# mwhoffman/pybo

Hardware: AMD Instinct MI355X
Metric: BO-step wall-clock (GP fit + 1e6-candidate acq sweep) at N obs; steps/sec (higher is better)
Workload: dtype f64

## Files before the change

### pybo_amd/csrc/api.hip

```cpp
#include <math.h>
#include <stdio.h>
#include <stdlib.h>
#include <string.h>

#include <algorithm>
#include <cmath>
#include <functional>
#include <new>
#include <type_traits>

#include "gpx_internal.h"
#include "gpx_diag.h"
#include "acq_core.h"
#include "ehvi_math.h"
#include "mes_math.h"
#include "kg_math.h"

using namespace gpx;

static thread_local std::string g_create_err;

#define HIPCHK(h, call)                                                                     \
    do {                                                                                    \
        hipError_t e_ = (call);                                                             \
// ... 93 lines not shown
}

enum { SHIP = 0, DIAG = 1 };
struct Option {
    const char* name;
    int diag;
    int64_t lo, hi;
    const char* bad;
    void (*set)(gpx_handle* h, int64_t v);
    bool (*ok)(int64_t v) = nullptr;
    const char* bad_ok = nullptr;
};
template <int gpx_handle::*F>
static void store(gpx_handle* h, int64_t v) { h->*F = (int)v; }
static bool mult128(int64_t v) { return v % 128 == 0; }
static const int64_t BIG = INT64_MAX;
static const char* const TG = "chol_tg*: out of range";
static const char* const TRTRI = "trtri_ahead*: out of range";
static const char* const XBG = "x_bg*: out of range";
static const Option kOptions[] = {
    {"chunk", SHIP, 128, BIG, "chunk must be a positive multiple of 128", [](gpx_handle* h, int64_t v) { h->chunk = v; }, mult128},
    {"super_m", SHIP, 1, 16, "super_m must be 1, 2, 4, 8 or 16", store<&gpx_handle::super_m>, [](int64_t v) { return (v & (v - 1)) == 0; }},
    {"tile_order", SHIP, -1, 31, "tile_order: -1 (by size) or bits 0-1 tile map (0..3), bits 2-4 k-loop schedule (1 .. 7)",
     store<&gpx_handle::tile_order>, [](int64_t v) { return v == -1 || v >= 4; }},
    {"sweep_cache", SHIP, -1, 1, "sweep_cache must be 1, 0 or -1",
     [](gpx_handle* h, int64_t v) { h->cache_on = (v == 1); if (v < 0) { h->cache_valid = false; h->npend = 0; } }},
    {"prune", SHIP, -1, 1, "prune must be -1 (by size and gate), 0 (never) or 1 (wherever legal)", store<&gpx_handle::prune>},
    {"prune_keep", DIAG, 0, 1, "prune_keep must be 0 or 1", store<&gpx_handle::prune_keep>},
    {"prune_bound", DIAG, -1, 2, "prune_bound must be -1 (by guard), 0 (generic kernel), 1 (matrix-pipe kernel) or 2 (fp32 matrix-pipe kernel)", store<&gpx_handle::prune_bound>},
    {"bound_fact", DIAG, 0, 1, "bound_fact must be 0 (the fp32 bound kernel never takes its factorised form) or 1 (by its guard)", store<&gpx_handle::bound_fact>},
    {"prune_rows", DIAG, -1, 1000000, "prune_rows must be -1 (by size), 0 (no second bound) or a number of block rows", store<&gpx_handle::prune_rows>},
    {"sweep_cols", SHIP, -1, 128, "sweep_cols must be -1 (by size), 128, 64 or 32", store<&gpx_handle::sweep_cols>,
     [](int64_t v) { return v == -1 || v == 128 || v == 64 || v == 32; }},
    {"prune_seeds", DIAG, 0, 1000000, "prune_seeds must be 0 (by the rule) or a number of seeds", store<&gpx_handle::prune_seeds>},
    {"short_map", DIAG, -1, 1, "short_map must be -1 (by size), 0 (never) or 1 (wherever tile map 3 is in use)", store<&gpx_handle::short_map>},
    {"chol_w", SHIP, 0, 8, "chol_w must be 0 (by size) or in [2, 8]", store<&gpx_handle::chol_w>, [](int64_t v) { return v != 1; }},
    {"chol_tg", SHIP, -1, 1000000000, TG, store<&gpx_handle::chol_tg>, [](int64_t v) { return v == 0 || v == 1; }, "chol_tg must be 0 or 1"},
    {"chol_tg_chunks", DIAG, -1, 1000000000, TG, store<&gpx_handle::tg_chunks>},
    {"chol_tg_grid", DIAG, -1, 1000000000, TG, store<&gpx_handle::tg_grid>},
    {"chol_tg_trace", DIAG, -1, 1000000000, TG, store<&gpx_handle::tg_trace>},
    {"chol_tg_isolate", DIAG, -1, 1000000000, TG, store<&gpx_handle::tg_isolate>},
    {"chol_tg_nap", DIAG, -1, 1000000000, TG, [](gpx_handle* h, int64_t v) { h->tg_nap = (int)std::max<int64_t>(0, std::min<int64_t>(127, v)); }},
    {"chol_tg_tmo_ms", SHIP, -1, 1000000000, TG, store<&gpx_handle::tg_tmo_ms>},
    {"chol_tg_min", SHIP, -1, 1000000000, TG, [](gpx_handle* h, int64_t v) { h->tg_min = (int)std::max<int64_t>(1, v); }},
    {"chol_tg_max", SHIP, -1, 1000000000, TG, [](gpx_handle* h, int64_t v) { h->tg_max = (int)std::max<int64_t>(1, v); }},
    {"chol_tg_db", SHIP, -1, 1000000000, TG, [](gpx_handle* h, int64_t v) { h->tg_db = (v < 0) ? -1 : (v != 0 ? 1 : 0); }},
    {"chol_tg_db_max", SHIP, -1, 1000000000, TG, [](gpx_handle* h, int64_t v) { h->tg_db_max = (int)std::max<int64_t>(0, v); }},
    {"chol_tg_fuse", SHIP, -1, 1000000000, TG, [](gpx_handle* h, int64_t v) { h->tg_fuse = (v != 0) ? 1 : 0; }},
    {"trtri_ahead", SHIP, 0, 1000000, TRTRI, [](gpx_handle* h, int64_t v) { h->trtri_ahead = (v != 0) ? 1 : 0; }},
    {"trtri_ahead_min", SHIP, 0, 1000000, TRTRI, [](gpx_handle* h, int64_t v) { h->trtri_ahead_min = (int)std::max<int64_t>(4, v); }},
    {"chol_fuse", SHIP, 0, 1, "chol_fuse must be 0 or 1", store<&gpx_handle::chol_fuse>},
    {"chol_graph", SHIP, 0, 1, "chol_graph must be 0 or 1", store<&gpx_handle::chol_graph>},
    {"chol_merge", SHIP, 0, 100000, "chol_merge: 0 (off) or a minimum number of block rows", store<&gpx_handle::chol_merge>},
    {"chol_rl", SHIP, 0, 1, "chol_rl must be 0 or 1", store<&gpx_handle::chol_rl>},
    {"x_skip", DIAG, 0, 7, "x_skip: bits 0..2", store<&gpx_handle::x_skip>},
    {"x_bg", DIAG, 0, 10000000, XBG, store<&gpx_handle::x_bg>},
    {"x_bg_lds", DIAG, 0, 10000000, XBG, store<&gpx_handle::x_bg_lds>},
    {"x_bg_iters", DIAG, 0, 10000000, XBG, store<&gpx_handle::x_bg_iters>},
    {"x_rff", DIAG, 0, 1, "x_rff must be 0 (by size) or 1 (the round-3 kernel)", [](gpx_handle*, int64_t v) { gpx::g_rff_variant = (int)v; }},
    {"grad_form", SHIP, 0, 2, "grad_form must be 0 (auto), 1 (two passes) or 2 (one pass)", store<&gpx_handle::grad_form>},
    {"grad_rb_cs", DIAG, 0, 65536, "grad_rb_cs must be a multiple of 128 (0 = default)", store<&gpx_handle::grad_rb_cs>, mult128},
    {"grad_kernel", SHIP, -1, 1, "grad_kernel must be -1 (auto), 0 or 1", store<&gpx_handle::grad_kernel>},
    {"trtri_left", SHIP, 0, 1, "trtri_left must be 0 or 1", store<&gpx_handle::trtri_left>},
    {"refine_inverse", SHIP, 0, 1, "refine_inverse must be 0 or 1", [](gpx_handle* h, int64_t v) { h->refine_inverse = (v != 0); }},
    {"eager_inverse", SHIP, 0, 1, "eager_inverse must be 0 or 1", [](gpx_handle* h, int64_t v) { h->eager_inverse = (v != 0); }},
};
// ... 968 lines not shown
        if (list.idx != w.idx) launch_sel_remap(s, w.idx, list.idx, list.n);
        launch_sel_scatter(s, list.idx, vals, list.n, out, nullptr);
    }
    *done = M;
    return GPX_OK;
}

static int plain_rest(const SelectOps& ops, const double* dXc, int64_t done, int64_t chunk, int64_t M, double* out, double* mu, double* s2) {
    const int64_t chunk1 = std::min(chunk, M);
    int rc;
    if (done > 0 && done < chunk1) {
        if ((rc = ops.exact(dXc, done, chunk1, out, mu, s2))) return rc;
        done = chunk1;
    }
    return done < M ? ops.exact(dXc, done, M, out, mu, s2) : GPX_OK;
}

static int second_bound(gpx_handle* h, const PruneWs& w, int64_t chunk, int sweep_order, double p0, SelectList& list) {
    hipStream_t s = h->stream;
    gpx_handle::PruneRecord& rec = h->prune_rec;
    const int64_t Np = h->Np, M = rec.M, Gg = rec.Gg, cap = rec.cap, nsurv = list.n;
    const int nP = (int)(Np / NB);
    int nR = 0;
    if (h->prune_rows > 0) nR = (int)std::min<int64_t>(std::min<int64_t>(h->prune_rows, nP), h->N / NB);
    else if (h->prune_rows < 0 && M >= PRUNE_MIN_M && nP >= PRUNE_ROWS_MIN_NP && nsurv > Gg) nR = std::max(1, nP / PRUNE_ROWS_DIV);
    if (nR <= 0 || nsurv <= 0) return GPX_OK;
    int64_t nsurv2 = 0;
    {
        Span sp(h, T_BOUND);
        for (int64_t j0 = 0; j0 < nsurv; j0 += chunk) {
            const int64_t valid = std::min(chunk, nsurv - j0);
            const int64_t cols = (valid + TBH - 1) / TBH * TBH;
            launch_cross_gram(s, h->dXs, (int64_t)nR * NB, h->N, (int)h->d, w.Xg, j0, nsurv, cols, h->dinvell, h->kernel_id, h->rho, h->dKs, Np);
            launch_sweep_trmm(s, h->dU, Np, nR, h->dKs, chunk, cols, h->da, h->dQp, h->dPp, chunk, sweep_order, h->super_m, h->dclk, h->short_map);
            launch_prune_ub2(s, h->dQp, chunk, nR, j0, valid, w.idx, w.dots, w.sc, h->rho, h->bias, p0, w.ub2, h->prune_keep ? w.qR : nullptr);
        }
    }
    {
        Span sp(h, T_ACQ);
        launch_sel_compact(s, w.ub2, nsurv, 1, w.st, w.sc + 5, w.blk2, cap, w.Xg, (int)h->d, w.idx2, w.Xg2);
        HIPCHK(h, hipMemcpyAsync(&nsurv2, w.blk2 + sel_blocks(nsurv), 8, hipMemcpyDeviceToHost, s));
    }
    HIPCHK(h, hipStreamSynchronize(s));
    rec.nR = nR, rec.nsurv2 = nsurv2;
    rec.ub2 = w.ub2, rec.idx2 = w.idx2, rec.qR = h->prune_keep ? w.qR : nullptr;
    list = {w.Xg2, w.idx2, nsurv2};
    return GPX_OK;
}

static int sweep_core(gpx_handle* h, int acq_id, const double* params, int nparams, const double* dXc,
                      int64_t M, int64_t k, double* top_val, int64_t* top_idx, double* d_acq,
                      double* d_mu, double* d_s2) {
    h->prune_rec = gpx_handle::PruneRecord();
    if (!h->fitted) return fail(h, GPX_ESTATE, "sweep: model is not fitted");
    if (!dXc || M < 1) return fail(h, GPX_EARG, "sweep: need M >= 1 candidates");
    int rc;
    if ((rc = check_acq(h, "sweep", acq_id, params, nparams, 0, true)) || (rc = check_topk(h, "sweep", k, top_val, top_idx))) return rc;
    HIPCHK(h, hipSetDevice(h->device));
    if ((rc = ensure_inverse(h))) return rc;
    hipStream_t s = h->stream;
    const int64_t Np = h->Np;
    const int nP = (int)(Np / NB);
    const int64_t chunk = sweep_chunk(h, M);
    if ((rc = ensure(h, h->dKs, h->cap_ks, Np * chunk))) return rc;
    if ((rc = ensure(h, h->dQp, h->cap_part, (int64_t)nP * chunk * 2))) return rc;
    h->dPp = h->dQp + (int64_t)nP * chunk;
    const bool selection_only = !d_acq && !d_mu && !d_s2;
// ... 9 lines not shown
    if (kg) {
        if ((rc = kg_prepare(h, params, nparams / (int)h->d, kb))) return rc;
        if ((rc = ensure(h, h->dkgw, h->cap_kgw, (int64_t)NB * chunk))) return rc;
    }
    double* cq = nullptr;
    double* cp = nullptr;
    if (h->cache_on) {
        spec_cancel(h);
        h->cache_valid = false;
        h->npend = 0;
        if ((rc = ensure(h, h->dcZ, h->cap_cz, M * h->d))) return rc;
        if ((rc = ensure(h, h->dcq, h->cap_cq, 2 * M))) return rc;
        h->dcp = h->dcq + h->cap_cq / 2;
        cq = h->dcq;
        cp = h->dcp;
        if (dXc != h->dcZ)
            HIPCHK(h, hipMemcpyAsync(h->dcZ, dXc, (size_t)M * h->d * 8, hipMemcpyDeviceToDevice, s));
    }

    const int sweep_order = h->tile_order >= 0 ? h->tile_order : (Np / NB < 32 ? 7 : 19);

    auto run_chunks = [&](const double* X, int64_t mb, int64_t me, double* out, double* mu, double* s2) -> int {
        for (int64_t m0 = mb; m0 < me; m0 += chunk) {
            const int64_t valid = std::min(chunk, me - m0);
            const int64_t cols = (valid + TBH - 1) / TBH * TBH;
            {
                Span sp(h, T_XGRAM);
                launch_cross_gram(s, h->dXs, Np, h->N, (int)h->d, X, m0, me, cols, h->dinvell, h->kernel_id,
                                  h->rho, h->dKs, Np);
            }
            {
                Span sp(h, T_TRMM);
                launch_sweep_trmm(s, h->dU, Np, nP, h->dKs, chunk, cols, h->da, h->dQp, h->dPp, chunk, sweep_order, h->super_m, h->dclk, h->short_map,
                                  valid, h->sweep_cols);
            }
            h->tacc[T_NLAUNCH] += 1.0;
            h->tacc[T_FLOP] += (double)h->N * (double)h->N * (double)valid;
            {
                Span sp(h, T_ACQ);
                if (kg) {
                    launch_kg_cross(s, kb.B, Np, h->dKs, Np, cols, h->dkgw, chunk);
                    launch_acq_kg(s, h->dQp, h->dPp, chunk, nP, m0, valid, h->rho, h->bias, h->sn2, h->kernel_id, (int)h->d, X, h->dinvell,
                                  kb.As, kb.m, kb.al, h->dkgw, chunk, out, mu, s2, cq, cp);
                } else if (mes) launch_acq_mes(s, h->dQp, h->dPp, chunk, nP, m0, valid, h->rho, h->bias, ys, out, mu, s2, cq, cp);
                else launch_acq(s, h->dQp, h->dPp, chunk, nP, m0, valid, h->rho, h->bias, acq_id, p0, out, mu, s2, cq, cp);
            }
        }
        return GPX_OK;
    };

    gpx_handle::PruneRecord& rec = h->prune_rec;
    PruneWs w;
    KeepWs kw = {};
    SelectOps ops;
    ops.exact = run_chunks;
    ops.gate = [&](int64_t Gg, double* value, bool* go) -> int {
        run_chunks(dXc, 0, Gg, d_acq, nullptr, w.gs2);
        launch_prune_mean(s, w.gs2, Gg, w.sc + 4);
        double mean_s2 = 0.0;
        HIPCHK(h, hipMemcpyAsync(&mean_s2, w.sc + 4, 8, hipMemcpyDeviceToHost, s));
        HIPCHK(h, hipStreamSynchronize(s));
        *go = mean_s2 >= h->rho * PRUNE_GATE_S2;
        *value = mean_s2;
        return GPX_OK;
    };
    ops.bound = [&](double* ub, int64_t done) -> int {
        const bool bound_mfma = h->prune_bound != 0 && bound_mfma_ks(h->kernel_id, (int)h->d) > 0;
// ... 1216 lines not shown
```

### pybo_amd/csrc/gemm_core.h

```cpp
#pragma once
#include <hip/hip_runtime.h>
#include <stdint.h>
#include <type_traits>

namespace gpx {

typedef double d4 __attribute__((ext_vector_type(4)));
typedef double d2 __attribute__((ext_vector_type(2)));

constexpr int TB = 128;
constexpr int BK = 16;
constexpr int LDT = TB + 16;
constexpr int GEMM_THREADS = 256;
constexpr int GEMM_LDS_F64 = 2 * 2 * BK * LDT;
constexpr int GEMM_LDS_BYTES = GEMM_LDS_F64 * 8;

template <int NJ>
__device__ __forceinline__ void acc_zero(d4 (&acc)[4][NJ]) {
#pragma unroll
    for (int i = 0; i < 4; ++i)
#pragma unroll
        for (int j = 0; j < NJ; ++j) acc[i][j] = (d4){0.0, 0.0, 0.0, 0.0};
}

// ... 473 lines not shown
        };
        frag(0, 0);
#pragma unroll
        for (int kk = 0; kk < G; ++kk) {
            if (kk + 1 < G) {
                frag((kk + 1) & 1, kk + 1);
                __builtin_amdgcn_sched_group_barrier(0x100, 8, 0);
            }
#pragma unroll
            for (int i = 0; i < 4; ++i)
#pragma unroll
                for (int j = 0; j < 4; ++j)
                    acc[i][j] = __builtin_amdgcn_mfma_f64_16x16x4f64(a[kk & 1][i], b[kk & 1][j], acc[i][j], 0, 0, NEGA ? 1 : 0);
            __builtin_amdgcn_sched_group_barrier(0x008, 16, 0);
            if (FILL && kk < 4) {
                if (kk == 0) issue(img, std::integral_constant<int, 0>{}, std::integral_constant<int, 2>{});
                if (kk == 1) issue(img, std::integral_constant<int, 2>{}, std::integral_constant<int, 4>{});
                if (kk == 2) issue(img, std::integral_constant<int, 4>{}, std::integral_constant<int, 6>{});
                if (kk == 3) issue(img, std::integral_constant<int, 6>{}, std::integral_constant<int, 8>{});
                __builtin_amdgcn_sched_group_barrier(0x020, 4, 0);
            }
        }
        asm volatile("" ::: "memory");
        if (FILL) {
            bump();
            asm volatile("s_waitcnt vmcnt(0) lgkmcnt(0)" ::: "memory");
            __builtin_amdgcn_s_barrier();
        }
    };
    int kt = 0;
    for (; kt + 1 < nk; ++kt) step(kt, std::true_type{});
    step(kt, std::false_type{});
    if (PRIO) __builtin_amdgcn_s_setprio(PRIO - 1);
    __builtin_amdgcn_s_barrier();
}

constexpr int GEMM_W_IMG_F64 = 2 * 16 * 64;

template <int NIMG, int PRIO = 1, bool NEGA = false, bool ILV = false, int AUX = 0, bool TRI = false>
__device__ __forceinline__ void gemm_tile_128_w(d4 (&acc)[4][4], const double* __restrict__ A, int64_t lda,
                                                const double* __restrict__ B, int64_t ldb, int k_lo, int k_hi,
                                                double* smem) {
    constexpr int BKW = 16, G = 4;
    const int lane = threadIdx.x & 63;
    const int w = __builtin_amdgcn_readfirstlane(threadIdx.x >> 6);
    const int wm = w >> 1, wn = w & 1;
    const int nk = (k_hi - k_lo) / BKW;
    if (nk <= 0) return;
    double* mine = smem + w * (NIMG * GEMM_W_IMG_F64);
    const char* Abase = reinterpret_cast<const char*>(A + (int64_t)k_lo * lda);
    const char* Bbase = reinterpret_cast<const char*>(B + (int64_t)k_lo * ldb);
    const int lp = lane >> 4, lr = (lane >> 3) & 1, lc = lane & 7;
    const int colA = (ILV ? (2 * lp + wm) * 16 : wm * 64 + 16 * lp) + 2 * lc, colB = wn * 64 + 16 * lp + 2 * lc;
    const int voA = (int)(((int64_t)lr * lda + colA) * 8), voB = (int)(((int64_t)lr * ldb + colB) * 8);
    const int soA = (int)(2 * lda * 8), soB = (int)(2 * ldb * 8);
    auto issue = [&](int img, auto q0c, auto q1c) {
        constexpr int Q0 = decltype(q0c)::value, Q1 = decltype(q1c)::value;
        double* As = mine + img * GEMM_W_IMG_F64;
        double* Bs = As + 16 * 64;
        __amdgpu_buffer_rsrc_t rA = __builtin_amdgcn_make_buffer_rsrc((void*)Abase, 0, -1, 0x00020000);
        __amdgpu_buffer_rsrc_t rB = __builtin_amdgcn_make_buffer_rsrc((void*)Bbase, 0, -1, 0x00020000);
#pragma unroll
        for (int q = Q0; q < Q1; ++q) {
            __builtin_amdgcn_raw_ptr_buffer_load_lds(rA, (gemm_lds_ptr)(As + q * 128), 16, voA, q * soA, 0, AUX);
            __builtin_amdgcn_raw_ptr_buffer_load_lds(rB, (gemm_lds_ptr)(Bs + q * 128), 16, voB, q * soB, 0, AUX);
        }
// ... 178 lines not shown
```

### pybo_amd/csrc/gpx_internal.h

```cpp
#pragma once
#include <hip/hip_runtime.h>
#include <stdint.h>
#include <string>
#include <vector>

#include "../../include/gpx.h"
#include "prune_hint.h"
#include "ws_layout.h"

namespace gpx {

constexpr int DMAX_RFF = DMAX;
constexpr int DMAX_RFF_RESIDENT = 64;
constexpr int TOPK_MAX = 4096;
constexpr int TOPK_PASS = 64;

enum Timer {
    T_GRAM = 0, T_CHOL, T_TRTRI, T_ALPHA, T_XGRAM, T_TRMM, T_ACQ, T_RFF, T_NLAUNCH, T_FLOP, T_COPY, T_APPEND,
    T_RANK1, T_RFFSWEEP, T_RFFOPS, T_TGFALL, T_SCLK, T_RFFCLK, T_AHEAD, T_BOUND, T_BATCH, T_JOINT, T_COUNT
};

struct EventPair { hipEvent_t a, b; int slot; };

struct EnsBatchMember {
    const double *cq, *cp, *invell;
    double *qp, *V, *cross, *scal, *xs;
    double rho, bias, sn2;
};

}

struct CholGraphKey {
    int64_t Np;
    int w, rl, merge, fuse;
    const void *S, *R, *T, *U, *flag;
    hipStream_t s2, s3, s4;
};

struct gpx_handle {
    int device = 0;
// ... 116 lines not shown
        int64_t M = 0, k = 0, G = 0, Gg = 0, done = 0, cap = 0, nsurv = 0;
        double gate = 0.0;
        bool hinted = false;
        const double* ub = nullptr;
        const int64_t* idx = nullptr;
        const double* sc = nullptr;
    };
    struct PruneRecord : SelectRecord {
        const int* st = nullptr;
        int bound_kernel = -1;
        bool kept = false;
        int nR = 0;
        int64_t nsurv2 = 0;
        const double *qR = nullptr, *ub2 = nullptr;
        const int64_t* idx2 = nullptr;
    } prune_rec;
    struct EnsPruneRecord : SelectRecord {
        int n = 0;
        const double* delta = nullptr;
    } ens_rec;
    struct ConPruneRecord : SelectRecord {
        int nc = 0;
    } con_rec;
    gpx::PruneHint prune_hint, ens_hint;
    int prune_keep = 0;
    int prune_bound = -1;
#ifdef GPX_BOUND32_NOFACT
    int bound_fact = 0;
#else
    int bound_fact = 1;
#endif
    int prune_rows = -1;
    int sweep_cols = -1;
    int prune_seeds = 0;
    int short_map = -1;
    char* dkeep = nullptr;
    int64_t cap_keep = 0;

    const double* app_w = nullptr;
    bool cache_on = false;
    bool cache_valid = false;
    int64_t cache_M = 0;
    double* dcZ = nullptr;
    double* dcq = nullptr;
    double* dcp = nullptr;
    int64_t cap_cz = 0, cap_cq = 0;
    double* dpend = nullptr;
    int64_t pend_ld = 0;
    int npend = 0;

    bool spec_active = false;
    bool spec_launched = false;
    bool spec_used = false;
    bool apply_pending = false;
    uint64_t gen = 0, spec_gen = 0;
    std::vector<double> spec_x;
    double* dspec = nullptr;
    int64_t cap_spec = 0, spec_ld = 0, spec_M = 0;
    hipEvent_t ev_spec_go = nullptr, ev_spec_done = nullptr;

    double* dbsel = nullptr;
    int64_t cap_bsel = 0;
    std::vector<gpx::EnsBatchMember> bsel_desc;

    double* djoint = nullptr;
    int64_t cap_joint = 0;
// ... 20 lines not shown

int ensure_bytes(gpx_handle* h, void** p, int64_t* cap, int64_t need, size_t elem, const char* what);
template <typename T> inline int ensure(gpx_handle* h, T*& p, int64_t& cap, int64_t need, const char* what = nullptr) {
    return ensure_bytes(h, reinterpret_cast<void**>(&p), &cap, need, sizeof(T), what);
}

void launch_scale_x(hipStream_t s, const double* X, int64_t n, int64_t np, int d, const double* invell,
                    double* Xs);
void launch_gram_sym(hipStream_t s, const double* Xs, int64_t N, int64_t Np, int d, int kernel_id,
                     double rho, double sn2, double* S);
int ensure_side_streams(gpx_handle* h);
void launch_cholesky(gpx_handle* h);
bool launch_cholesky_tg(gpx_handle* h);
int tg_abort_code(gpx_handle* h);
int64_t tg_trace_copy(gpx_handle* h, long long* out, int64_t n);
void tg_free(gpx_handle* h);
int64_t tg_tasks_copy(int nP, int chunks, int16_t* out, int64_t cap, int64_t* counts);
void launch_trtri(gpx_handle* h);
void launch_trtri_ahead(gpx_handle* h, hipStream_t s, int top);
int trtri_top(int nP);
void launch_refine_inverse(gpx_handle* h, double* tmp);
void launch_alpha(gpx_handle* h);
void launch_kinv_diag(gpx_handle* h, double* out);
void launch_transpose_lower(hipStream_t s, const double* R, int64_t Np, double* out, int64_t N);
void launch_cholesky_small(hipStream_t s, double* S, double* R, int64_t np, int* flag);
void launch_posterior_wide(hipStream_t s, const double* A, const double* v, const double* z, int n, int64_t np, double sc,
                           double sn2, double* B, double* R, double* work, int* flag, double* theta);

void launch_cross_gram(hipStream_t s, const double* Xs, int64_t rows, int64_t N, int d, const double* Xc,
                       int64_t m0, int64_t M, int64_t cols, const double* invell, int kernel_id,
                       double rho, double* Ks, int64_t ldk);
void launch_sweep_trmm(hipStream_t s, const double* U, int64_t Np, int nR, const double* Ks, int64_t ldk,
                       int64_t cols, const double* a, double* Qp, double* Pp, int64_t ldp,
                       int tile_order, int super_m, unsigned long long* clk, int short_map = -1, int64_t valid = -1, int sweep_cols = 128);
int sweep_cols_of(int sweep_cols, int tile_order, int nP, int nR, int64_t valid);
constexpr int SWEEP_NARROW_MIN_NP = 48;
void launch_acq(hipStream_t s, const double* Qp, const double* Pp, int64_t ldp, int nrb, int64_t m0,
                int64_t cols_valid, double rho, double bias, int acq_id, double p0, double* acq_out,
                double* mu_out, double* s2_out, double* qsum, double* psum);
struct MesArg;
void launch_acq_mes(hipStream_t s, const double* Qp, const double* Pp, int64_t ldp, int nrb, int64_t m0,
                    int64_t cols_valid, double rho, double bias, const MesArg& ys, double* acq_out,
                    double* mu_out, double* s2_out, double* qsum, double* psum);
void launch_kg_solve(hipStream_t s, const double* U, int64_t Np, int64_t N, int m, const double* V, double* W);
void launch_kg_cross(hipStream_t s, const double* B, int64_t Np, const double* Ks, int64_t ldk, int64_t cols, double* C, int64_t ldc);
void launch_acq_kg(hipStream_t s, const double* Qp, const double* Pp, int64_t ldp, int nrb, int64_t m0, int64_t cols_valid,
                   double rho, double bias, double sn2, int kid, int d, const double* X, const double* invell, const double* As, int m,
                   const double* al, const double* C, int64_t ldc, double* acq_out, double* mu_out, double* s2_out, double* qsum,
                   double* psum);
void launch_kg_point_sums(hipStream_t s, const double* Xs, int64_t N, int d, const double* Z, int np, const double* invell, int kid,
                          double rho, const double* B, const double* alpha, const double* Wz, const double* Vz, double* S);
void launch_kg_point_final(hipStream_t s, const double* S, int np, int d, const double* Z, const double* invell, const double* As,
                           int m, const double* al, int kid, double rho, double bias, double sn2, double* L, double* f, double* g);
void launch_pend_store(hipStream_t s, const double* w, int64_t Nj, int64_t ldw, const double* scal, double* row,
                       double* pscal_j);
void launch_cache_apply(hipStream_t s, const double* v, const double* scal, int64_t M, double* qsum, double* psum);
void launch_scale_point(hipStream_t s, const double* x, const double* invell, int d, double* xs);
void launch_sweep_rank1_v(hipStream_t s, const double* Xs, int64_t Ntot, int d, const double* Wq, int64_t ldw,
                          const double* pscal, const double* Z, int64_t M, const double* invell, int kernel_id,
                          double rho, const double* xlast, double* vout, const double* skip = nullptr);
void launch_sweep_rankq(hipStream_t s, const double* Xs, int64_t Ntot, int d, const double* Wq, int64_t ldw, int q,
                        const double* pscal, const double* Z, int64_t M, const double* invell, int kernel_id,
                        double rho, double* qsum, double* psum);
void launch_topk(hipStream_t s, const double* vals, int64_t M, int k, double* blkv, int64_t* blki,
                 int64_t nblk, double* topv, int64_t* topi);
void launch_topk_merge(hipStream_t s, double* vals, int64_t* idx, int64_t n, int k, double* topv, int64_t* topi);
void launch_topk_rows(hipStream_t s, const double* vals, int64_t M, int64_t S, int k, double* blkv, int64_t* blki,
                      int64_t nblk, double* topv, int64_t* topi);
void launch_prune_alpha(hipStream_t s, const double* U, int64_t Np, const double* a, double rho, double bias, double* alpha2,
// ... 92 lines not shown
```

### pybo_amd/csrc/kernels_sweep.hip

```cpp
#include "acq_core_dev.h"
#include "gemm_core.h"
#include "gpx_internal.h"
#include "gpx_math.h"
#include "bound_exp.h"
#include "bound_f32.h"
#include "sweep_map.h"

namespace gpx {

constexpr int XK = 64, XN = 128, XDC = 16;

template <bool FIRST>
__device__ __forceinline__ void dist_step(const double (*xo)[XK], const double (*xc)[XN], int k, int ty, int tx,
                                          double (&r2)[8][4]) {
    double a8[8], b4[4];
#pragma unroll
    for (int a = 0; a < 8; ++a) a8[a] = xo[k][ty * 8 + a];
#pragma unroll
    for (int b = 0; b < 4; ++b) b4[b] = xc[k][tx * 4 + b];
#pragma unroll
    for (int a = 0; a < 8; ++a)
#pragma unroll
        for (int b = 0; b < 4; ++b) {
            const double df = a8[a] - b4[b];
// ... 164 lines not shown
                                                                int order, int sm, unsigned long long* clk) {
    __shared__ __attribute__((aligned(16))) double smem[GEMM_LDS_F64];
    sweep_tiles<64>(blockIdx.x, U, Np, Ks, NT, nR, avec, Qp, Pp, ldp, order, sm, clk, smem,
                    [&](d4 (&acc)[4][4], const double* At, const double* Bt, int kend, bool rev, int) {
        if (!rev) {
            if (VAR == 2) gemm_tile_128_b<true, true>(acc, At, Np, Bt, TB, 0, kend, smem);
            else if (VAR == 5) gemm_tile_128_g<1, false, true>(acc, At, Np, Bt, TB, 0, kend, smem);
            else gemm_tile_128_s<1, false, true>(acc, At, Np, Bt, TB, 0, kend, smem);
        } else {
            if (VAR == 2) gemm_rev32(0, kend, [&](int k0, int k1) { gemm_tile_128_b<true, true>(acc, At, Np, Bt, TB, k0, k1, smem); });
            else if (VAR == 5) gemm_tile_128_g<1, false, true, true>(acc, At, Np, Bt, TB, 0, kend, smem);
            else gemm_tile_128_s<1, false, true, true>(acc, At, Np, Bt, TB, 0, kend, smem);
        }
    });
}

template <int BKL, int WGS, int PRIO, int NSET, bool TRI, int AUX = 0, bool DOWN = true, int NJ = 4>
__global__ __launch_bounds__(GEMM_THREADS, WGS) void k_sweep_trmm_l(const double* __restrict__ U, int64_t Np,
                                                                    const double* __restrict__ Ks, int64_t ldk, int NT, int nR,
                                                                    const double* __restrict__ avec,
                                                                    double* __restrict__ Qp, double* __restrict__ Pp,
                                                                    int64_t ldp, int order, int sm,
                                                                    unsigned long long* clk, int b0) {
    __shared__ __attribute__((aligned(16))) double smem[gemm_l_lds_f64<BKL>()];
    static_assert(NJ == 4 || BKL == 32, "narrow tiles: the 32-row k-step only");
    sweep_tiles<32 * WGS, NJ>((int)blockIdx.x + b0, U, Np, Ks, NT, nR, avec, Qp, Pp, ldp, order, sm, clk, smem,
                              [&](d4 (&acc)[4][NJ], const double* At, const double* Bt, int kend, bool rev, int bcol) {
        if (!(DOWN && rev)) gemm_tile_128_l<BKL, PRIO, NSET, true, TRI, false, AUX>(acc, At, Np, Bt, TB, 0, kend, smem, bcol);
        else if constexpr (BKL == 32) gemm_tile_128_l<32, PRIO, NSET, true, TRI, false, AUX, true>(acc, At, Np, Bt, TB, 0, kend, smem, bcol);
        else gemm_rev32(0, kend, [&](int k0, int k1) { gemm_tile_128_l<BKL, PRIO, NSET, true, false, false, AUX>(acc, At, Np, Bt, TB, k0, k1, smem); });
    });
}

__global__ __launch_bounds__(GEMM_THREADS, 2) void k_sweep_trmm_w(const double* __restrict__ U, int64_t Np,
                                                                  const double* __restrict__ Ks, int64_t ldk, int NT, int nR,
                                                                  const double* __restrict__ avec, double* __restrict__ Qp,
                                                                  double* __restrict__ Pp, int64_t ldp, int order, int sm,
                                                                  unsigned long long* clk) {
    __shared__ __attribute__((aligned(16))) double smem[4 * GEMM_W_IMG_F64];
    sweep_tiles<64>(blockIdx.x, U, Np, Ks, NT, nR, avec, Qp, Pp, ldp, order, sm, clk, smem,
                    [&](d4 (&acc)[4][4], const double* At, const double* Bt, int kend, bool rev, int) {
        if (!rev) gemm_tile_128_w<1, 1, false, true, 0, true>(acc, At, Np, Bt, TB, 0, kend, smem);
        else gemm_rev32(0, kend, [&](int k0, int k1) { gemm_tile_128_w<1, 1, false, true, 0, false>(acc, At, Np, Bt, TB, k0, k1, smem); });
    });
}

template <int RES>
static int sweep_order_of(int order, int short_map, int sm, int NT) {
    if (order != 3 || short_map == 0) return order;
    if (short_map < 0 && !sweep_map_is_short<RES>(sm, NT)) return order;
    return short_map == 2 ? SWEEP_ORDER_SHORT_STRIDED : SWEEP_ORDER_SHORT;
}

static const int64_t SWEEP_COLS32_MAX = 512, SWEEP_COLS64_MAX = 1024;
int sweep_cols_of(int sweep_cols, int tile_order, int nP, int nR, int64_t valid) {
    if (tile_order < 0 || ((tile_order >> 2) & 7) != 4 || (tile_order >> 5) != 0) return TB;
    if (sweep_cols > 0) return sweep_cols;
    if (nP < SWEEP_NARROW_MIN_NP || nR != nP || (tile_order & 3) != 3) return TB;
    return valid <= SWEEP_COLS32_MAX ? 32 : valid <= SWEEP_COLS64_MAX ? 64 : TB;
}

void launch_sweep_trmm(hipStream_t s, const double* U, int64_t Np, int nR, const double* Ks, int64_t ldk,
                       int64_t cols, const double* a, double* Qp, double* Pp, int64_t ldp,
                       int tile_order, int super_m, unsigned long long* clk, int short_map, int64_t valid, int sweep_cols) {
    const int NT = (int)(cols / TB);
    if (valid < 0 || valid > cols) valid = cols;
    const int order0 = tile_order & 3, var = (tile_order >> 2) & 7;
#define GPX_SW(K) hipLaunchKernelGGL(K, dim3(nblk), dim3(GEMM_THREADS), 0, s, U, Np, Ks, ldk, NT, nR, a, Qp, Pp, ldp, order, super_m, clk)
#define GPX_SWL(K) hipLaunchKernelGGL(K, dim3(nblk), dim3(GEMM_THREADS), 0, s, U, Np, Ks, ldk, NT, nR, a, Qp, Pp, ldp, order, super_m, clk, 0)
    if (var == 7) {
        const int order = sweep_order_of<96>(order0, short_map, super_m, NT);
        const unsigned nblk = sweep_grid<96>(order, super_m, NT, nR);
        GPX_SWL((k_sweep_trmm_l<16, 3, 1, 2, false>));
    } else if (var == 1) {
        const int order = sweep_order_of<64>(order0, short_map, super_m, NT);
        const unsigned nblk = sweep_grid<64>(order, super_m, NT, nR);
        GPX_SW(k_sweep_trmm_w);
    } else if (const int W = sweep_cols_of(sweep_cols, tile_order, (int)(Np / TB), nR, valid); W < TB) {
        const int NTn = (int)((valid + W - 1) / W);
        const int order = sweep_order_of<64>(order0, short_map, super_m, NTn);
        const unsigned nblk = sweep_grid<64>(order, super_m, NTn, nR);
#define GPX_SWN(K) hipLaunchKernelGGL(K, dim3(nblk), dim3(GEMM_THREADS), 0, s, U, Np, Ks, ldk, NTn, nR, a, Qp, Pp, ldp, order, super_m, clk, 0)
        if (W == 64) GPX_SWN((k_sweep_trmm_l<32, 2, 1, 2, true, 0, true, 2>));
        else GPX_SWN((k_sweep_trmm_l<32, 2, 1, 2, true, 0, true, 1>));
#undef GPX_SWN
    } else if (var == 4 || var == 3) {
        const int order = sweep_order_of<64>(order0, short_map, super_m, NT);
        const unsigned nblk = sweep_grid<64>(order, super_m, NT, nR);
#ifdef GPX_SWEEP_PROBES
        const int aux = tile_order >> 5;
        if (var == 4 && aux == 1) GPX_SWL((k_sweep_trmm_l<32, 2, 1, 2, true, 1>));
        else if (var == 4 && aux == 2) GPX_SWL((k_sweep_trmm_l<32, 2, 1, 2, true, 2>));
        else if (var == 4 && aux == 3) GPX_SWL((k_sweep_trmm_l<32, 2, 1, 2, true, 16>));
        else if (var == 4 && aux == 4) GPX_SWL((k_sweep_trmm_l<32, 2, 1, 2, true, 17>));
        else if (var == 4 && aux == 5) GPX_SWL((k_sweep_trmm_l<32, 2, 1, 2, true, 3>));
        else if (var == 4 && aux == 6) GPX_SWL((k_sweep_trmm_l<32, 2, 1, 2, true, 0, false>));
        else if (var == 4 && aux == 7) {
            for (unsigned g0 = 0; g0 < nblk; g0 += 512)
                hipLaunchKernelGGL((k_sweep_trmm_l<32, 2, 1, 2, true>), dim3(nblk - g0 < 512 ? nblk - g0 : 512), dim3(GEMM_THREADS), 0, s, U, Np, Ks, ldk, NT, nR, a,
                                   Qp, Pp, ldp, order, super_m, clk, (int)g0);
        }
        else
#endif
        if (var == 4) GPX_SWL((k_sweep_trmm_l<32, 2, 1, 2, true>));
        else GPX_SWL((k_sweep_trmm_l<32, 2, 1, 2, false>));
    } else {
        const int order = sweep_order_of<64>(order0, short_map, super_m, NT);
        const unsigned nblk = sweep_grid<64>(order, super_m, NT, nR);
        if (var == 2) GPX_SW(k_sweep_trmm<2>);
        else if (var == 6) GPX_SW(k_sweep_trmm<6>);
        else GPX_SW(k_sweep_trmm<5>);
// ... 935 lines not shown
```

### pybo_amd/csrc/sweep_map.h

```cpp
#ifndef GPX_SWEEP_MAP_H
#define GPX_SWEEP_MAP_H

#if defined(__HIPCC__) || defined(__CUDACC__)
#define GPX_MAP_FN __host__ __device__ __forceinline__
#else
#define GPX_MAP_FN inline
#endif

namespace gpx {

constexpr int SWEEP_ORDER_SHORT = 4;
constexpr int SWEEP_ORDER_SHORT_STRIDED = 5;

template <int RES>
GPX_MAP_FN bool sweep_map_is_short(int sm, int NT) { return (NT + 7) / 8 < RES / sm; }

template <int RES>
GPX_MAP_FN bool sweep_short_share(int x, bool strided, int sm, int NT, int nR, int& p0, int& pstep, int& R, int& t0, int& W) {
    const int SN = RES / sm;
    const int P = (nR + 1) / 2;
    int xn_nat = 1;
    while (xn_nat < 8 && xn_nat * SN < NT) xn_nat *= 2;
    const int xm_nat = 8 / xn_nat;
    const int XM = xm_nat < P ? xm_nat : P;
// ... 70 lines not shown
        mt = nP - 1 - i;
        if (i < mt) mt2 = i;
        return true;
    }
    mt = nP - 1 - b / NT;
    nt = b - (b / NT) * NT;
    return true;
}

template <int RES>
GPX_MAP_FN unsigned sweep_grid(int order, int super_m, int NT, int nP) {
    const int per = (NT + 7) / 8;
    if (order == 1) return (unsigned)(8 * per * nP);
    if (order == 2 || order == 3) {
        const int SN = RES / super_m;
        const int hper = (per + SN - 1) / SN;
        const int rows = (order == 3) ? (nP + 1) / 2 : nP;
        const int gm = (rows + super_m - 1) / super_m;
        return (unsigned)(8 * RES * hper * gm);
    }
    if (order == SWEEP_ORDER_SHORT || order == SWEEP_ORDER_SHORT_STRIDED) {
        int dmax = 0, xlast = 0;
        for (int x = 0; x < 8; ++x) {
            int p0, pstep, R, t0, W;
            if (!sweep_short_share<RES>(x, order == SWEEP_ORDER_SHORT_STRIDED, super_m, NT, nP, p0, pstep, R, t0, W)) continue;
            const int dx = sweep_short_depth<RES>(super_m, R, W);
            if (dx >= dmax) { dmax = dx; xlast = x; }
        }
        return dmax ? (unsigned)(8 * (dmax - 1) + xlast + 1) : 0u;
    }
    return (unsigned)(NT * nP);
}

}
#endif
```

Before: 86.75.

## Add double-buffered LDS sweep TRMM kernel and size-based sweep shape selection

Adds a new sweep TRMM GEMM tile path that keeps two LDS images of each K-step, issuing the next step's buffer-to-LDS loads while the current step's MFMAs run. A new sweep_shape_of heuristic picks the column width and whether to use the two-image kernel, based on per-XCD tile load and the CU count. It also lets the second-bound prune pass choose narrower widths for prefix (nR<nP) sweeps. The aim is to hide global load latency and balance small sweeps across CUs, at the cost of larger dynamic LDS per block and more heuristic complexity.

```diff
diff --git a/pybo_amd/csrc/api.hip b/pybo_amd/csrc/api.hip
--- a/pybo_amd/csrc/api.hip
+++ b/pybo_amd/csrc/api.hip
@@ -149,6 +149,7 @@
     {"prune_rows", DIAG, -1, 1000000, "prune_rows must be -1 (by size), 0 (no second bound) or a number of block rows", store<&gpx_handle::prune_rows>},
     {"sweep_cols", SHIP, -1, 128, "sweep_cols must be -1 (by size), 128, 64 or 32", store<&gpx_handle::sweep_cols>,
      [](int64_t v) { return v == -1 || v == 128 || v == 64 || v == 32; }},
+    {"sweep_images", SHIP, -1, 2, "sweep_images must be -1 (by size), 1 or 2", store<&gpx_handle::sweep_images>, [](int64_t v) { return v != 0; }},
     {"prune_seeds", DIAG, 0, 1000000, "prune_seeds must be 0 (by the rule) or a number of seeds", store<&gpx_handle::prune_seeds>},
     {"short_map", DIAG, -1, 1, "short_map must be -1 (by size), 0 (never) or 1 (wherever tile map 3 is in use)", store<&gpx_handle::short_map>},
     {"chol_w", SHIP, 0, 8, "chol_w must be 0 (by size) or in [2, 8]", store<&gpx_handle::chol_w>, [](int64_t v) { return v != 1; }},
@@ -1183,7 +1184,8 @@
             const int64_t valid = std::min(chunk, nsurv - j0);
             const int64_t cols = (valid + TBH - 1) / TBH * TBH;
             launch_cross_gram(s, h->dXs, (int64_t)nR * NB, h->N, (int)h->d, w.Xg, j0, nsurv, cols, h->dinvell, h->kernel_id, h->rho, h->dKs, Np);
-            launch_sweep_trmm(s, h->dU, Np, nR, h->dKs, chunk, cols, h->da, h->dQp, h->dPp, chunk, sweep_order, h->super_m, h->dclk, h->short_map);
+            launch_sweep_trmm(s, h->dU, Np, nR, h->dKs, chunk, cols, h->da, h->dQp, h->dPp, chunk, sweep_order, h->super_m, h->dclk, h->short_map,
+                              valid, h->sweep_cols, h->sweep_images);
             launch_prune_ub2(s, h->dQp, chunk, nR, j0, valid, w.idx, w.dots, w.sc, h->rho, h->bias, p0, w.ub2, h->prune_keep ? w.qR : nullptr);
         }
     }
@@ -1259,7 +1261,7 @@
             {
                 Span sp(h, T_TRMM);
                 launch_sweep_trmm(s, h->dU, Np, nP, h->dKs, chunk, cols, h->da, h->dQp, h->dPp, chunk, sweep_order, h->super_m, h->dclk, h->short_map,
-                                  valid, h->sweep_cols);
+                                  valid, h->sweep_cols, h->sweep_images);
             }
             h->tacc[T_NLAUNCH] += 1.0;
             h->tacc[T_FLOP] += (double)h->N * (double)h->N * (double)valid;
diff --git a/pybo_amd/csrc/gemm_core.h b/pybo_amd/csrc/gemm_core.h
--- a/pybo_amd/csrc/gemm_core.h
+++ b/pybo_amd/csrc/gemm_core.h
@@ -529,6 +529,117 @@
     for (; kt + 1 < nk; ++kt) step(kt, std::true_type{});
     step(kt, std::false_type{});
     if (PRIO) __builtin_amdgcn_s_setprio(PRIO - 1);
+    __builtin_amdgcn_s_barrier();
+}
+
+template <int PRIO = 1, int NSET = 2, bool ILV = false, bool TRI = false, bool NEGA = false, int AUX = 0, bool REV = false, int NJ = 4, int FG = (NJ == 1 ? 1 : 4)>
+__device__ __forceinline__ void gemm_tile_128_l2(d4 (&acc)[4][NJ], const double* __restrict__ A, int64_t lda,
+                                                 const double* __restrict__ B, int64_t ldb, int k_lo, int k_hi,
+                                                 double* smem, int bcol = 0) {
+    static_assert(NJ == 4 || NJ == 2 || NJ == 1, "a wave owns 4, 2 or 1 column groups");
+    static_assert(!TRI || ILV, "TRI needs the interleaved row blocks");
+    static_assert(FG == 1 || FG == 2 || FG == 4 || FG == 8, "the step's 16 DMA instructions in FG equal pieces");
+    constexpr int G = BK32 / 4;
+    constexpr int IMG = gemm_l_lds_f64<BK32>();
+    const int lane = threadIdx.x & 63;
+    const int w = __builtin_amdgcn_readfirstlane(threadIdx.x >> 6);
+    const int wm = w >> 1, wn = w & 1;
+    const int nk = (k_hi - k_lo) / BK32;
+    if (nk <= 0) return;
+    const char* Abase = reinterpret_cast<const char*>(A + (int64_t)(REV ? k_hi - BK32 : k_lo) * lda);
+    const char* Bbase = reinterpret_cast<const char*>(B + (int64_t)(REV ? k_hi - BK32 : k_lo) * ldb);
+    const int64_t stepA = (REV ? -1 : 1) * (int64_t)BK32 * lda * 8, stepB = (REV ? -1 : 1) * (int64_t)BK32 * ldb * 8;
+    const int voA = (int)(((int64_t)w * lda + 2 * lane) * 8), voB = (int)(((int64_t)w * ldb + 2 * lane) * 8);
+    const int soA = (int)(4 * lda * 8), soB = (int)(4 * ldb * 8);
+    auto issue = [&](int img, int p0, int p1) {
+        double* As = smem + img * IMG;
+        double* Bs = As + BK32 * LDT;
+        __amdgpu_buffer_rsrc_t rA = __builtin_amdgcn_make_buffer_rsrc((void*)Abase, 0, -1, 0x00020000);
+        __amdgpu_buffer_rsrc_t rB = __builtin_amdgcn_make_buffer_rsrc((void*)Bbase, 0, -1, 0x00020000);
+#pragma unroll
+        for (int p = p0; p < p1; ++p) {
+            __builtin_amdgcn_raw_ptr_buffer_load_lds(rA, (gemm_lds_ptr)(As + (w + 4 * p) * LDT), 16, voA, p * soA, 0, AUX);
+            __builtin_amdgcn_raw_ptr_buffer_load_lds(rB, (gemm_lds_ptr)(Bs + (w + 4 * p) * LDT), 16, voB, p * soB, 0, AUX);
+        }
+    };
+    auto bump = [&]() {
+        Abase += stepA;
+        Bbase += stepB;
+    };
+    const int fr = lane & 15, fk = lane >> 4;
+    constexpr int IST = ILV ? 32 : 16;
+    const int aoff = (ILV ? wm * 16 : wm * 64) + fr + fk * LDT;
+    const int boff = BK32 * LDT + bcol + wn * (16 * NJ) + fr + fk * LDT;
+    issue(0, 0, G);
+    bump();
+    asm volatile("s_waitcnt vmcnt(0)" ::: "memory");
+    __builtin_amdgcn_s_barrier();
+    if (PRIO) __builtin_amdgcn_s_setprio(PRIO);
+    int kt = 0;
+    auto step = [&](auto i0c, auto fillc) {
+        constexpr int I0 = decltype(i0c)::value;
+        constexpr bool FILL = decltype(fillc)::value;
+        const double* as = smem + (kt & 1) * IMG + aoff;
+        const double* bs = smem + (kt & 1) * IMG + boff;
+        const int img = (kt + 1) & 1;
+        asm volatile("" ::: "memory");
+        double a[NSET][4], b[NSET][NJ];
+        auto frag = [&](int set, int g) {
+#pragma unroll
+            for (int i = I0; i < 4; ++i) a[set][i] = as[g * 4 * LDT + i * IST];
+#pragma unroll
+            for (int j = 0; j < NJ; ++j) b[set][j] = bs[g * 4 * LDT + j * 16];
+        };
+        frag(0, 0);
+#pragma unroll
+        for (int kk = 0; kk < G; ++kk) {
+            if (NSET == 2 && kk + 1 < G) {
+                frag((kk + 1) & 1, kk + 1);
+                __builtin_amdgcn_sched_group_barrier(0x100, 4 + NJ - I0, 0);
+            }
+#pragma unroll
+            for (int i = I0; i < 4; ++i)
+#pragma unroll
+                for (int j = 0; j < NJ; ++j)
+                    acc[i][j] = __builtin_amdgcn_mfma_f64_16x16x4f64(a[kk % NSET][i], b[kk % NSET][j], acc[i][j], 0, 0, NEGA ? 1 : 0);
+            __builtin_amdgcn_sched_group_barrier(0x008, NJ * (4 - I0), 0);
+            if (FILL && kk < FG) {
+                issue(img, kk * (G / FG), (kk + 1) * (G / FG));
+                __builtin_amdgcn_sched_group_barrier(0x020, 2 * (G / FG), 0);
+            }
+            if (NSET == 1 && kk + 1 < G) frag(0, kk + 1);
+        }
+        asm volatile("" ::: "memory");
+        if (FILL) {
+            bump();
+            asm volatile("s_waitcnt vmcnt(0) lgkmcnt(0)" ::: "memory");
+            __builtin_amdgcn_s_barrier();
+        }
+        ++kt;
+    };
+    using T_ = std::true_type;
+    using F_ = std::false_type;
+    using I0_ = std::integral_constant<int, 0>;
+    if (!TRI) {
+        for (int t = 0; t + 1 < nk; ++t) step(I0_{}, T_{});
+        step(I0_{}, F_{});
+    } else {
+        const int nd = nk - 3;
+        if (!REV) {
+            for (int t = 0; t < nd; ++t) step(I0_{}, T_{});
+            step(std::integral_constant<int, 1>{}, T_{});
+            step(std::integral_constant<int, 2>{}, T_{});
+            step(std::integral_constant<int, 3>{}, F_{});
+        } else {
+            step(std::integral_constant<int, 3>{}, T_{});
+            step(std::integral_constant<int, 2>{}, T_{});
+            step(std::integral_constant<int, 1>{}, T_{});
+            for (int t = 0; t + 1 < nd; ++t) step(I0_{}, T_{});
+            step(I0_{}, F_{});
+        }
+    }
+    if (PRIO) __builtin_amdgcn_s_setprio(PRIO - 1);
+    asm volatile("s_waitcnt lgkmcnt(0)" ::: "memory");
     __builtin_amdgcn_s_barrier();
 }
 
diff --git a/pybo_amd/csrc/gpx_internal.h b/pybo_amd/csrc/gpx_internal.h
--- a/pybo_amd/csrc/gpx_internal.h
+++ b/pybo_amd/csrc/gpx_internal.h
@@ -6,6 +6,7 @@
 
 #include "../../include/gpx.h"
 #include "prune_hint.h"
+#include "sweep_map.h"
 #include "ws_layout.h"
 
 namespace gpx {
@@ -188,6 +189,7 @@
 #endif
     int prune_rows = -1;
     int sweep_cols = -1;
+    int sweep_images = -1;
     int prune_seeds = 0;
     int short_map = -1;
     char* dkeep = nullptr;
@@ -274,9 +276,8 @@
                        double rho, double* Ks, int64_t ldk);
 void launch_sweep_trmm(hipStream_t s, const double* U, int64_t Np, int nR, const double* Ks, int64_t ldk,
                        int64_t cols, const double* a, double* Qp, double* Pp, int64_t ldp,
-                       int tile_order, int super_m, unsigned long long* clk, int short_map = -1, int64_t valid = -1, int sweep_cols = 128);
-int sweep_cols_of(int sweep_cols, int tile_order, int nP, int nR, int64_t valid);
-constexpr int SWEEP_NARROW_MIN_NP = 48;
+                       int tile_order, int super_m, unsigned long long* clk, int short_map = -1, int64_t valid = -1, int sweep_cols = 128,
+                       int sweep_images = 1);
 void launch_acq(hipStream_t s, const double* Qp, const double* Pp, int64_t ldp, int nrb, int64_t m0,
                 int64_t cols_valid, double rho, double bias, int acq_id, double p0, double* acq_out,
                 double* mu_out, double* s2_out, double* qsum, double* psum);
diff --git a/pybo_amd/csrc/kernels_sweep.hip b/pybo_amd/csrc/kernels_sweep.hip
--- a/pybo_amd/csrc/kernels_sweep.hip
+++ b/pybo_amd/csrc/kernels_sweep.hip
@@ -220,6 +220,25 @@
     });
 }
 
+template <int NSET, int NJ, int FG = (NJ == 1 ? 1 : 4)>
+__global__ __launch_bounds__(GEMM_THREADS, 2) void k_sweep_trmm_l2(const double* __restrict__ U, int64_t Np,
+                                                                   const double* __restrict__ Ks, int64_t ldk, int NT, int nR,
+                                                                   const double* __restrict__ avec,
+                                                                   double* __restrict__ Qp, double* __restrict__ Pp,
+                                                                   int64_t ldp, int order, int sm,
+                                                                   unsigned long long* clk, int b0) {
+    extern __shared__ __attribute__((aligned(16))) double sweep_l2_smem[];
+    sweep_tiles<32, NJ>((int)blockIdx.x + b0, U, Np, Ks, NT, nR, avec, Qp, Pp, ldp, order, sm, clk, sweep_l2_smem,
+                        [&](d4 (&acc)[4][NJ], const double* At, const double* Bt, int kend, bool rev, int bcol) {
+        if (!rev) gemm_tile_128_l2<1, NSET, true, true, false, 0, false, NJ, FG>(acc, At, Np, Bt, TB, 0, kend, sweep_l2_smem, bcol);
+        else gemm_tile_128_l2<1, NSET, true, true, false, 0, true, NJ, FG>(acc, At, Np, Bt, TB, 0, kend, sweep_l2_smem, bcol);
+    });
+}
+constexpr int SWEEP_L2_LDS_BYTES = 2 * gemm_l_lds_f64<32>() * 8;
+#ifdef GPX_SWEEP_PROBES
+static int g_sweep_probe_fg = 0;
+#endif
+
 __global__ __launch_bounds__(GEMM_THREADS, 2) void k_sweep_trmm_w(const double* __restrict__ U, int64_t Np,
                                                                   const double* __restrict__ Ks, int64_t ldk, int NT, int nR,
                                                                   const double* __restrict__ avec, double* __restrict__ Qp,
@@ -233,26 +252,26 @@
     });
 }
 
-template <int RES>
-static int sweep_order_of(int order, int short_map, int sm, int NT) {
-    if (order != 3 || short_map == 0) return order;
-    if (short_map < 0 && !sweep_map_is_short<RES>(sm, NT)) return order;
-    return short_map == 2 ? SWEEP_ORDER_SHORT_STRIDED : SWEEP_ORDER_SHORT;
-}
-
-static const int64_t SWEEP_COLS32_MAX = 512, SWEEP_COLS64_MAX = 1024;
-int sweep_cols_of(int sweep_cols, int tile_order, int nP, int nR, int64_t valid) {
-    if (tile_order < 0 || ((tile_order >> 2) & 7) != 4 || (tile_order >> 5) != 0) return TB;
-    if (sweep_cols > 0) return sweep_cols;
-    if (nP < SWEEP_NARROW_MIN_NP || nR != nP || (tile_order & 3) != 3) return TB;
-    return valid <= SWEEP_COLS32_MAX ? 32 : valid <= SWEEP_COLS64_MAX ? 64 : TB;
+
+static int device_cus() {
+    static int cus[64] = {};
+    int dev = 0;
+    if (hipGetDevice(&dev) != hipSuccess || dev < 0 || dev >= 64) return 0;
+    if (!cus[dev]) {
+        int n = 0;
+        if (hipDeviceGetAttribute(&n, hipDeviceAttributeMultiprocessorCount, dev) != hipSuccess || n <= 0) return 0;
+        cus[dev] = n;
+    }
+    return cus[dev];
 }
 
 void launch_sweep_trmm(hipStream_t s, const double* U, int64_t Np, int nR, const double* Ks, int64_t ldk,
                        int64_t cols, const double* a, double* Qp, double* Pp, int64_t ldp,
-                       int tile_order, int super_m, unsigned long long* clk, int short_map, int64_t valid, int sweep_cols) {
+                       int tile_order, int super_m, unsigned long long* clk, int short_map, int64_t valid, int sweep_cols, int sweep_images) {
     const int NT = (int)(cols / TB);
     if (valid < 0 || valid > cols) valid = cols;
+    const SweepShape shape = sweep_shape_of(tile_order, (int)(Np / TB), nR, valid, sweep_images < 0 ? device_cus() : 0, sweep_cols, sweep_images,
+                                            super_m, short_map);
     const int order0 = tile_order & 3, var = (tile_order >> 2) & 7;
 #define GPX_SW(K) hipLaunchKernelGGL(K, dim3(nblk), dim3(GEMM_THREADS), 0, s, U, Np, Ks, ldk, NT, nR, a, Qp, Pp, ldp, order, super_m, clk)
 #define GPX_SWL(K) hipLaunchKernelGGL(K, dim3(nblk), dim3(GEMM_THREADS), 0, s, U, Np, Ks, ldk, NT, nR, a, Qp, Pp, ldp, order, super_m, clk, 0)
@@ -264,7 +283,30 @@
         const int order = sweep_order_of<64>(order0, short_map, super_m, NT);
         const unsigned nblk = sweep_grid<64>(order, super_m, NT, nR);
         GPX_SW(k_sweep_trmm_w);
-    } else if (const int W = sweep_cols_of(sweep_cols, tile_order, (int)(Np / TB), nR, valid); W < TB) {
+    } else if (shape.images == 2) {
+        const int W = shape.width;
+        const int NTn = (int)((valid + W - 1) / W);
+        const int order = sweep_order_of<32>(order0, short_map, super_m, NTn);
+        const unsigned nblk = sweep_grid<32>(order, super_m, NTn, nR);
+#define GPX_SW2(K)                                                                                                        \
+    do {                                                                                                                  \
+        hipFuncSetAttribute((const void*)K, hipFuncAttributeMaxDynamicSharedMemorySize, SWEEP_L2_LDS_BYTES);              \
+        hipLaunchKernelGGL(K, dim3(nblk), dim3(GEMM_THREADS), SWEEP_L2_LDS_BYTES, s, U, Np, Ks, ldk, NTn, nR, a, Qp, Pp, ldp, order, super_m, clk, 0); \
+    } while (0)
+#ifdef GPX_SWEEP_PROBES
+        const int fg = (int)g_sweep_probe_fg;
+        if (W == 32 && fg == 2) GPX_SW2((k_sweep_trmm_l2<2, 1, 2>));
+        else if (W == 32 && fg == 4) GPX_SW2((k_sweep_trmm_l2<2, 1, 4>));
+        else if (W == 64 && fg == 2) GPX_SW2((k_sweep_trmm_l2<2, 2, 2>));
+        else if (W == 64 && fg == 1) GPX_SW2((k_sweep_trmm_l2<2, 2, 1>));
+        else if (W == 128 && fg == 1) GPX_SW2((k_sweep_trmm_l2<2, 4, 1>));
+        else
+#endif
+        if (W == 32) GPX_SW2((k_sweep_trmm_l2<2, 1>));
+        else if (W == 64) GPX_SW2((k_sweep_trmm_l2<2, 2>));
+        else GPX_SW2((k_sweep_trmm_l2<2, 4>));
+#undef GPX_SW2
+    } else if (const int W = shape.width; W < TB) {
         const int NTn = (int)((valid + W - 1) / W);
         const int order = sweep_order_of<64>(order0, short_map, super_m, NTn);
         const unsigned nblk = sweep_grid<64>(order, super_m, NTn, nR);
diff --git a/pybo_amd/csrc/sweep_map.h b/pybo_amd/csrc/sweep_map.h
--- a/pybo_amd/csrc/sweep_map.h
+++ b/pybo_amd/csrc/sweep_map.h
@@ -126,5 +126,71 @@
     return (unsigned)(NT * nP);
 }
 
+template <int RES>
+GPX_MAP_FN int sweep_order_of(int order, int short_map, int sm, int NT) {
+    if (order != 3 || short_map == 0) return order;
+    if (short_map < 0 && !sweep_map_is_short<RES>(sm, NT)) return order;
+    return short_map == 2 ? SWEEP_ORDER_SHORT_STRIDED : SWEEP_ORDER_SHORT;
+}
+
+constexpr int SWEEP_NARROW_MIN_NP = 48;
+constexpr long long SWEEP_COLS32_MAX = 512, SWEEP_COLS64_MAX = 1024;
+constexpr int SWEEP_PREFIX_MIN_W = 32;
+struct SweepShape { int width, images; };
+
+GPX_MAP_FN long long sweep_working(int order, int NT, int nR) { return (long long)NT * (order == 3 ? (nR + 1) / 2 : nR); }
+
+template <int RES>
+GPX_MAP_FN long long sweep_xcd_load(int short_map, int sm, int NT, int nR) {
+    const int P = (nR + 1) / 2;
+    const int order = sweep_order_of<RES>(3, short_map, sm, NT);
+    long long worst = 0;
+    for (int x = 0; x < 8; ++x) {
+        long long wx;
+        if (order == 3) {
+            const int per = (NT + 7) / 8;
+            const int t0 = x * per;
+            wx = (long long)P * (t0 >= NT ? 0 : (NT - t0 < per ? NT - t0 : per));
+        } else {
+            int p0, pstep, R, t0, W;
+            wx = sweep_short_share<RES>(x, order == SWEEP_ORDER_SHORT_STRIDED, sm, NT, nR, p0, pstep, R, t0, W) ? (long long)R * W : 0;
+        }
+        if (wx > worst) worst = wx;
+    }
+    return worst;
+}
+
+GPX_MAP_FN long long sweep_prefix_cost(int short_map, int sm, int nR, long long valid, int W) {
+    const long long load = sweep_xcd_load<64>(short_map, sm, (int)((valid + W - 1) / W), nR);
+    const long long rem = load % 64;
+    const long long units = load / 64 * 20 + (rem == 0 ? 0 : rem <= 32 ? 12 : 20);
+    return units * (W / 32) * (W == 128 ? 100 : W == 64 ? 105 : 115);
+}
+GPX_MAP_FN int sweep_prefix_width(int short_map, int sm, int nR, long long valid) {
+    int best = 128;
+    long long best_cost = sweep_prefix_cost(short_map, sm, nR, valid, 128);
+    for (int W = 64; W >= SWEEP_PREFIX_MIN_W; W /= 2) {
+        const long long cost = sweep_prefix_cost(short_map, sm, nR, valid, W);
+        if (cost * 100 < best_cost * 95) best = W, best_cost = cost;
+    }
+    return best;
+}
+
+GPX_MAP_FN SweepShape sweep_shape_of(int tile_order, int nP, int nR, long long valid, int cus, int sweep_cols, int sweep_images, int sm,
+                                     int short_map) {
+    SweepShape s = {128, 1};
+    if (tile_order < 0 || ((tile_order >> 2) & 7) != 4 || (tile_order >> 5) != 0) return s;
+    const int order0 = tile_order & 3;
+    const bool by_size = nP >= SWEEP_NARROW_MIN_NP && order0 == 3;
+    if (sweep_cols > 0) s.width = sweep_cols;
+    else if (by_size) s.width = nR != nP ? sweep_prefix_width(short_map, sm, nR, valid) : valid <= SWEEP_COLS32_MAX ? 32 : valid <= SWEEP_COLS64_MAX ? 64 : 128;
+    if (sweep_images > 0) s.images = sweep_images;
+    else if (by_size) {
+        const int NT = (int)((valid + s.width - 1) / s.width);
+        if (sweep_working(order0, NT, nR) <= cus && 8 * sweep_xcd_load<32>(short_map, sm, NT, nR) <= cus) s.images = 2;
+    }
+    return s;
+}
+
 }
 #endif
```

Measured after the change: 89.91, median of 6. 1.04x the previous value.
